# noahchalifour/rnnt-speech-recognition

Measured on AMD Instinct MI355X. Metric: rnnt_loss_grad_lattice_cells_per_sec, higher is better.
Workload: dtype f32

## Files before the change

rnnt-speech-recognition_amd/csrc/rnnt_common.h:

```cpp
#pragma once
#include <hip/hip_runtime.h>
#include <stdint.h>

#include <type_traits>

namespace rnnt {

constexpr float kNeg = -1.0e30f;
constexpr float kNegTest = -1.0e29f;
constexpr float kLog2e = 1.4426950408889634f;
constexpr float kLn2 = 0.6931471805599453f;
constexpr int kRebase = 8;

struct FastDiv {
    uint32_t d, m, s;
};
inline FastDiv make_fastdiv(uint32_t d) {
    FastDiv f;
    f.d = d;
    uint32_t s = 0;
    while ((1ull << s) < d) ++s;
    f.s = s;
    f.m = (uint32_t)((((1ull << s) - d) << 32) / d) + 1u;
    return f;
}
__device__ __forceinline__ uint32_t fdiv(uint32_t n, const FastDiv f) {
    return (__umulhi(n, f.m) + n) >> f.s;
}

struct TileGeom {
    int TT, UU, tiles_t, tiles_u, cpr;
    FastDiv div_tu, div_tt, divUU, div_cpr, divTT;
};

struct LossParams {
    const float *acts;
    float *grads;
    const int *labels;
    const int *label_lengths;
    const int *input_lengths;
    const float *cost_scale;
    float *costs;
    float *lse;
    float *W;
    float *A;
    float *Bt;
    float *offA;
    float *offB;
    double *ll;
    int *EA;
    int *EB;
    float *lik;
    int *flags;
    int NCl;
    float2 *pstat;
    int *lshift;
    int *bar;
    int nPstat;
    int pstatStride;
    int B, T, U, V, blank;
    int b0, nb;
    int visit_all;
    int precise;
    int N, Nr, Up, NC, NG;
    uint32_t cells;
    FastDiv divU, divT, divV, divOG;
    TileGeom tile;
    float fe_lambda;
};

struct WsLayout {
    size_t lse, W, A, Bt, offA, offB, ll, EA, EB, lik, flags, pstat, lshift, bar, total;
    int NCl, nPstat;
    int N, Nr, Up, NC, NG, OG;
};

inline size_t align_up(size_t x, size_t a) { return (x + a - 1) / a * a; }

constexpr int kMaxU = 8192;
inline int sweep_K(int U) {
    const int k = (U + 63) / 64;
    const int avail[] = {1, 2, 3, 4, 6, 8, 12, 16};
    for (int a : avail)
        if (k <= a) return a;
    return 0;
}
template <int K, int G>
struct SweepRing {
    static constexpr size_t kChunk = (size_t)G * 2 * 64 * K * sizeof(float);
    static constexpr int NB = (4 * kChunk + 16 <= 128 * 1024) ? 4 : 3;
    static constexpr size_t kBytes = NB * kChunk + 16;
    static_assert(kBytes <= 160 * 1024, "chunk ring exceeds the LDS");
};
template <typename F>
inline hipError_t sweep_dispatch(int U, F &&f) {
    using std::integral_constant;
    switch (sweep_K(U)) {
        case 1: return f(integral_constant<int, 1>(), integral_constant<int, 16>());
        case 2: return f(integral_constant<int, 2>(), integral_constant<int, 16>());
        case 3: return f(integral_constant<int, 3>(), integral_constant<int, 16>());
        case 4: return f(integral_constant<int, 4>(), integral_constant<int, 16>());
        case 6: return f(integral_constant<int, 6>(), integral_constant<int, 8>());
        case 8: return f(integral_constant<int, 8>(), integral_constant<int, 8>());
        case 12: return f(integral_constant<int, 12>(), integral_constant<int, 4>());
        case 16: return f(integral_constant<int, 16>(), integral_constant<int, 4>());
        default: return hipErrorInvalidValue;
    }
}
constexpr int kFillByte = 0xF1;

inline WsLayout make_layout(int T, int U, int B) {
    WsLayout w;
    w.N = T + U - 1;
    w.Nr = (int)align_up((size_t)w.N, 16);
    w.Up = sweep_K(U) ? 64 * sweep_K(U) : (int)align_up((size_t)U, 64);
    w.NC = w.Nr / kRebase + 1;
    w.OG = sweep_K(U) ? sweep_K(U) : 64;
    w.NG = w.Up / w.OG;
    size_t off = 0;
    auto take = [&](size_t bytes) {
        size_t o = off;
        off = align_up(off + bytes, 256);
        return o;
    };
    w.lse = take((size_t)B * T * U * sizeof(float));
    w.W = take((size_t)B * w.Nr * 2 * w.Up * sizeof(float));
    w.A = take((size_t)B * w.Nr * w.Up * sizeof(float));
    w.Bt = take((size_t)B * w.Nr * w.Up * sizeof(float));
    w.offA = take((size_t)B * w.NC * w.NG * sizeof(float));
    w.offB = take((size_t)B * w.NC * w.NG * sizeof(float));
    w.ll = take((size_t)B * 2 * sizeof(double));
    w.NCl = w.Nr / 4 + 1;
    w.EA = take((size_t)B * w.NCl * 64 * sizeof(int));
    w.EB = take((size_t)B * w.NCl * 64 * sizeof(int));
    w.lik = take((size_t)B * 4 * sizeof(float));
    w.flags = take((size_t)B * 4 * sizeof(int));
    {
        const int nu = (U + 31) / 32, UU = (U + nu - 1) / nu, TT = (256 / UU) > T ? T : (256 / UU);
        w.nPstat = ((T + TT - 1) / TT) * ((U + UU - 1) / UU) * 4;
    }
    w.pstat = take((size_t)B * w.nPstat * 2 * sizeof(float));
    w.lshift = take((size_t)B * sizeof(int));
    w.bar = take((size_t)B * 8 * sizeof(int));
    w.total = off;
    return w;
}

inline TileGeom make_tile(int T, int U, int V) {
    TileGeom g;
    const int nu = (U + 31) / 32;
    g.UU = (U + nu - 1) / nu;
    g.TT = 256 / g.UU;
    if (g.TT > T) g.TT = T;
    g.tiles_u = (U + g.UU - 1) / g.UU;
    g.tiles_t = (T + g.TT - 1) / g.TT;
    g.cpr = g.UU * V / 4;
    g.div_tu = make_fastdiv((uint32_t)g.tiles_u);
    g.div_tt = make_fastdiv((uint32_t)g.tiles_t);
    g.divUU = make_fastdiv((uint32_t)g.UU);
    g.divTT = make_fastdiv((uint32_t)(g.TT > 0 ? g.TT : 1));
    g.div_cpr = make_fastdiv((uint32_t)(g.cpr > 0 ? g.cpr : 1));
    return g;
}

constexpr float kExpTabLimit = 43.0f;
constexpr float kExpTab2Log2e = 2.8853900817779268f;
#ifdef __HIPCC__
__device__ __forceinline__ float exp_tab(float x) { return __builtin_amdgcn_exp2f(x * kExpTab2Log2e); }
__device__ __forceinline__ bool exp_tab_out_of_range(float x) { return !(fabsf(x) <= kExpTabLimit); }
#endif

constexpr int kHookBlocks = 1024;
struct JointHooks {
    int prep_mode;
    int prefilled;
    unsigned *dmax_enc;
    unsigned *dmax_pred;
};

#ifdef __HIPCC__
__device__ __forceinline__ void lds_dma16(const void *global, void *lds) {
    __builtin_amdgcn_global_load_lds((__attribute__((address_space(1))) const void *)global, (__attribute__((address_space(3))) void *)lds, 16, 0, 0);
}
#endif

inline int device_cu_count() {
    int dev = 0, n = 0;
    if (hipGetDevice(&dev) != hipSuccess) return 256;
    if (hipDeviceGetAttribute(&n, hipDeviceAttributeMultiprocessorCount, dev) != hipSuccess || n <= 0) return 256;
    return n;
}
template <typename Kernel>
inline hipError_t set_lds(Kernel kernel, size_t bytes) {
    if (bytes <= 64 * 1024) return hipSuccess;
    return hipFuncSetAttribute((const void *)kernel, hipFuncAttributeMaxDynamicSharedMemorySize, (int)bytes);
}

hipError_t launch_fill(void *dst, int byte, size_t bytes, hipStream_t s);
hipError_t launch_fill2(void *dst0, int byte0, size_t bytes0, void *dst1, int byte1, size_t bytes1, hipStream_t s);

bool tile_path_ok(const LossParams &p, bool grad);
hipError_t launch_lsm(const LossParams &p, hipStream_t s);
hipError_t launch_sweeps(const LossParams &p, hipStream_t s);
hipError_t launch_grad(const LossParams &p, hipStream_t s);
bool lin_path_ok(const LossParams &p);
hipError_t launch_lsm_lin(const LossParams &p, hipStream_t s);
hipError_t launch_sweeps_lin(const LossParams &p, hipStream_t s);
hipError_t launch_grad_lin(const LossParams &p, hipStream_t s);
hipError_t launch_redo_lin(const LossParams &p, bool force, hipStream_t s);

}
```

rnnt-speech-recognition_amd/csrc/rnnt_entrypoint.hip:

```cpp
#include "../../include/rnnt.h"
#include "rnnt_common.h"
#include "rnnt_lin.h"
#include "rnnt_align.h"
#include "rnnt_host.h"

using namespace rnnt;

namespace rnnt {
hipError_t joint_workspace_bytes(int T, int U, int B, int J, int V, int joint_dtype, size_t *bytes);
hipError_t joint_f16_backward_rows(void *workspace, int T, int U, int B, int J, int V, int rows[2], hipStream_t s);
hipError_t joint_backward_rows(void *workspace, int T, int U, int B, int J, int V, int rows[2], hipStream_t s);
hipError_t launch_joint_loss(const float *enc_proj, const float *pred_proj, const float *W2, const float *b2,
                             const int *labels, const int *label_lengths, const int *input_lengths,
                             const float *cost_scale, int J, int V, int B, int T, int U, int blank, float *costs,
                             float *d_enc_proj, float *d_pred_proj, float *dW2, float *db2, int joint_dtype,
                             int phases, void *workspace, hipStream_t s, const JointHooks *hooks, float fe_lambda);
hipError_t joint_aux_pointers(void *workspace, int T, int U, int B, int J, int V, float **expE, float **expP, float **tflag);
hipError_t launch_joint_prefill(void *workspace, int T, int U, int B, int J, int V, hipStream_t s);
bool joint_dtype_supported(int joint_dtype, int J, int V);
bool dense_supported(int H, int J);
hipError_t dense_workspace_bytes(int B, int T, int U, int H, int J, size_t base, size_t *bytes);
void dense_proj_pointers(void *workspace, int B, int T, int U, int H, int J, size_t base, float **enc_proj, float **pred_proj,
                         float **d_enc_proj, float **d_pred_proj);
void dense_hook_pointers(void *workspace, int B, int T, int U, int H, int J, size_t base, unsigned **dmax_enc, unsigned **dmax_pred);
// ... 27 lines not shown
                                    int Tc, int K, int N, int joint_dtype, bool timed, void *workspace, hipStream_t s);
hipError_t launch_beam_stream_feed(const float *enc, int Te, const int *chunk_frames, const int *reset, const int *final_, int H, int J,
                                   int V, int S, int Tc, int K, int N, int joint_dtype, bool timed, void *workspace, hipStream_t s);
bool prednet_layout_ok(const rnntPrednetBlock *blocks, int L, int E, int V, int Jp, int R, size_t *bytes);
hipError_t launch_prednet_begin(const float *emb, const rnntPrednetBlock *blocks, int L, int E, int V, const float *W1, int Jp, int R,
                                float *out, void *workspace, hipStream_t s);
hipError_t launch_prednet_step(const int *emitted, const int *parents, float *out, const rnntPrednetBlock *blocks, int L, int E,
                               int V, int Jp, int R, void *workspace, hipStream_t s);
bool encoder_layout_ok(const rnntPrednetBlock *blocks, int L, int F, float bn_eps, int ridx, int f, int R, int Tmax, size_t *bytes);
hipError_t launch_encoder_begin(const rnntPrednetBlock *blocks, int L, int F, const float *bn_mean, const float *bn_var,
                                const float *bn_weight, const float *bn_bias, float bn_eps, int ridx, int f, int R, int Tmax,
                                void *workspace, hipStream_t s);
hipError_t launch_encoder_run(const float *x, int T, float *out, const rnntPrednetBlock *blocks, int L, int F, float bn_eps, int ridx,
                              int f, int R, int Tmax, void *workspace, hipStream_t s);
hipError_t launch_encoder_run_rows(const float *x, int T, const int *row_frames, const int *reset, float *out,
                                   const rnntPrednetBlock *blocks, int L, int F, float bn_eps, int ridx, int f, int R, int Tmax,
                                   void *workspace, hipStream_t s);
bool lstm_train_layout_ok(int R, int T, int H, int P, bool proj, size_t *bytes);
hipError_t launch_lstm_train_fwd(float *gates, const float *W_hh, const float *W_hr, float *y, float *c, float *h, int R, int T, int H,
                                 int P, void *workspace, hipStream_t s);
hipError_t launch_lstm_train_bwd(float *gates, const float *c, const float *dy, const float *W_hh, const float *W_hr, float *dr, int R,
                                 int T, int H, int P, void *workspace, hipStream_t s);
hipError_t launch_prednet_reset(const int *reset, float *out, const rnntPrednetBlock *blocks, int L, int E, int V, int Jp, int R,
                                void *workspace, hipStream_t s);
hipError_t greedy_stream_workspace_bytes(int Tc, int S, int H, int J, int V, int joint_dtype, size_t *bytes);
hipError_t launch_greedy_stream_begin(const float *W1, const float *b1, const float *W2, const float *b2, int H, int J, int V, int S,
                                      int Tc, int joint_dtype, void *workspace, hipStream_t s);
hipError_t launch_greedy_stream_feed(const float *enc, int Te, const int *chunk_frames, const int *reset, const int *final_,
                                     const int *max_symbols, int max_per_frame, int *hyp_lengths, float *scores, int *all_done,
                                     int *frame_base, int H, int J, int V, int S, int Tc, int joint_dtype, void *workspace,
                                     hipStream_t s);
bool frontend_layout_ok(int K, int S, int L, int step, int M, int stack, int rm, size_t *bytes, int *max_rows);
hipError_t launch_frontend_begin(const float *window, const float *mel_weights, int K, int S, int L, int step, int M, int stack,
                                 int rm, void *workspace, hipStream_t s);
hipError_t launch_frontend_feed(const float *audio, int cs, const int *samples, const int *reset, const int *final_, int norm,
                                float *rows, int *counts, int K, int S, int L, int step, int M, int stack, int rm, void *workspace,
                                hipStream_t s);
}

static rnntStatus_t check_options(const rnntOptions &o) {
    if (o.loc != RNNT_GPU) return RNNT_STATUS_INVALID_VALUE;
    if (!o.batch_first) return RNNT_STATUS_INVALID_VALUE;
    if (o.maxT <= 0 || o.maxU <= 0 || o.blank_label < 0) return RNNT_STATUS_INVALID_VALUE;
    if (o.maxU > kMaxU) return RNNT_STATUS_INVALID_VALUE;
    return RNNT_STATUS_SUCCESS;
}

static bool fill_params(LossParams &p, const float *acts, float *grads, const int *labels,
                        const int *label_lengths, const int *input_lengths, const float *cost_scale, int V,
                        int B, float *costs, void *workspace, const rnntOptions &o) {
    const long long cells = (long long)B * o.maxT * o.maxU;
    if (cells <= 0 || cells >= (1ll << 31)) return false;
    if (((uintptr_t)workspace & 255) != 0) return false;
    const WsLayout w = make_layout(o.maxT, o.maxU, B);
    char *ws = (char *)workspace;
    p.acts = acts;
    p.grads = grads;
    p.labels = labels;
    p.label_lengths = label_lengths;
    p.input_lengths = input_lengths;
    p.cost_scale = cost_scale;
    p.costs = costs;
    p.lse = (float *)(ws + w.lse);
    p.W = (float *)(ws + w.W);
    p.A = (float *)(ws + w.A);
    p.Bt = (float *)(ws + w.Bt);
    p.offA = (float *)(ws + w.offA);
    p.offB = (float *)(ws + w.offB);
    p.ll = (double *)(ws + w.ll);
    p.EA = (int *)(ws + w.EA);
    p.EB = (int *)(ws + w.EB);
    p.lik = (float *)(ws + w.lik);
    p.flags = (int *)(ws + w.flags);
    p.NCl = w.NCl;
    p.pstat = (float2 *)(ws + w.pstat);
    p.lshift = (int *)(ws + w.lshift);
    p.bar = (int *)(ws + w.bar);
    p.nPstat = w.nPstat;
    p.pstatStride = 4;
    p.B = B, p.T = o.maxT, p.U = o.maxU, p.V = V, p.blank = o.blank_label;
    p.b0 = 0, p.nb = B;
    p.precise = 0;
    p.visit_all = 0;
    p.fe_lambda = 0.f;
    p.tile = make_tile(o.maxT, o.maxU, V);
    p.N = w.N, p.Nr = w.Nr, p.Up = w.Up, p.NC = w.NC, p.NG = w.NG;
    p.cells = (uint32_t)cells;
    p.divU = make_fastdiv((uint32_t)o.maxU);
    p.divT = make_fastdiv((uint32_t)o.maxT);
    p.divV = make_fastdiv((uint32_t)V);
    p.divOG = make_fastdiv((uint32_t)w.OG);
    return true;
}

namespace rnnt {
bool fill_loss_params(LossParams &p, const float *acts, float *grads, const int *labels, const int *label_lengths,
                      const int *input_lengths, const float *cost_scale, int V, int B, float *costs, void *workspace,
                      int maxT, int maxU, int blank) {
    rnntOptions o;
    o.loc = RNNT_GPU, o.stream = nullptr, o.blank_label = blank, o.maxT = maxT, o.maxU = maxU, o.batch_first = true;
    return fill_params(p, acts, grads, labels, label_lengths, input_lengths, cost_scale, V, B, costs, workspace, o);
}
}

extern "C" {

int get_warprnnt_version(void) { return 1; }

const char *rnntGetStatusString(rnntStatus_t status) {
    switch (status) {
        case RNNT_STATUS_SUCCESS: return "no error";
        case RNNT_STATUS_MEMOPS_FAILED: return "hip memcpy or memset failed";
        case RNNT_STATUS_INVALID_VALUE: return "invalid value";
        case RNNT_STATUS_EXECUTION_FAILED: return "execution failed";
        case RNNT_STATUS_UNKNOWN_ERROR:
        default: return "unknown error";
    }
}

rnntStatus_t get_workspace_size(int maxT, int maxU, int minibatch, bool gpu, size_t *size_bytes) {
    if (!size_bytes || maxT <= 0 || maxU <= 0 || minibatch <= 0 || !gpu) return RNNT_STATUS_INVALID_VALUE;
    *size_bytes = make_layout(maxT, maxU, minibatch).total;
    return RNNT_STATUS_SUCCESS;
}

static rnntStatus_t run_forward(LossParams &p, const WsLayout &w, hipStream_t s) {
    if (lin_path_ok(p)) {
        hipError_t e = launch_lsm_lin(p, s);
        if (e != hipSuccess) return from_hip(e);
        return from_hip(launch_sweeps_lin(p, s));
    }
    if (!tile_path_ok(p, false) && launch_fill(p.W, kFillByte, w.A - w.W, s) != hipSuccess) return RNNT_STATUS_MEMOPS_FAILED;
    p.precise = 1;
    hipError_t e = launch_lsm(p, s);
    if (e != hipSuccess) return from_hip(e);
    return from_hip(launch_sweeps(p, s));
}

static rnntStatus_t validate(const void *acts, const void *labels, const void *ll, const void *il, const void *ws,
                      int V, int B, const rnntOptions &o) {
    if (!acts || !labels || !ll || !il || !ws) return RNNT_STATUS_INVALID_VALUE;
    if (V <= 0 || B <= 0) return RNNT_STATUS_INVALID_VALUE;
    rnntStatus_t st = check_options(o);
    if (st != RNNT_STATUS_SUCCESS) return st;
    if (o.blank_label >= V) return RNNT_STATUS_INVALID_VALUE;
    return RNNT_STATUS_SUCCESS;
}

rnntStatus_t compute_rnnt_loss_fwd(const float *acts, const int *flat_labels, const int *label_lengths,
                                   const int *input_lengths, int alphabet_size, int minibatch, float *costs,
                                   void *workspace, rnntOptions options) {
    if (!costs) return RNNT_STATUS_INVALID_VALUE;
    rnntStatus_t st = validate(acts, flat_labels, label_lengths, input_lengths, workspace, alphabet_size, minibatch,
                               options);
    if (st != RNNT_STATUS_SUCCESS) return st;
    LossParams p;
    if (!fill_params(p, acts, nullptr, flat_labels, label_lengths, input_lengths, nullptr, alphabet_size,
                     minibatch, costs, workspace, options))
        return RNNT_STATUS_INVALID_VALUE;
    hipStream_t s = (hipStream_t)options.stream;
    const WsLayout w = make_layout(options.maxT, options.maxU, minibatch);
    st = run_forward(p, w, s);
    if (st != RNNT_STATUS_SUCCESS || !lin_path_ok(p)) return st;
    return from_hip(launch_redo_lin(p, false, s));
}

static rnntStatus_t run_backward(LossParams &p, hipStream_t s) {
    if (!lin_path_ok(p)) return from_hip(launch_grad(p, s));
    const bool patch = tile_path_ok(p, true);
    if (patch) {
        hipError_t e = launch_grad_lin(p, s);
        if (e != hipSuccess) return from_hip(e);
    }
    return from_hip(launch_redo_lin(p, !patch, s));
}

rnntStatus_t compute_rnnt_loss_bwd(const float *acts, float *grads, const int *flat_labels,
                                   const int *label_lengths, const int *input_lengths, const float *cost_scale,
                                   int alphabet_size, int minibatch, void *workspace, rnntOptions options) {
    if (!grads) return RNNT_STATUS_INVALID_VALUE;
    rnntStatus_t st = validate(acts, flat_labels, label_lengths, input_lengths, workspace, alphabet_size, minibatch,
                               options);
    if (st != RNNT_STATUS_SUCCESS) return st;
    LossParams p;
    if (!fill_params(p, acts, grads, flat_labels, label_lengths, input_lengths, cost_scale, alphabet_size,
                     minibatch, nullptr, workspace, options))
        return RNNT_STATUS_INVALID_VALUE;
    return run_backward(p, (hipStream_t)options.stream);
}

static bool fastemit_ok(float lambda) { return lambda >= 0.f && lambda <= 1.f; }

static rnntStatus_t loss_flags_call(const float *acts, float *grads, const int *flat_labels,
                                    const int *label_lengths, const int *input_lengths, const float *cost_scale,
                                    int alphabet_size, int minibatch, float *costs, void *workspace,
                                    const rnntOptions &options, unsigned int flags, float fastemit_lambda) {
    if (flags & ~(unsigned)RNNT_VISIT_ALL) return RNNT_STATUS_INVALID_VALUE;
    if (!grads)
        return compute_rnnt_loss_fwd(acts, flat_labels, label_lengths, input_lengths, alphabet_size, minibatch,
                                     costs, workspace, options);
    rnntStatus_t st = validate(acts, flat_labels, label_lengths, input_lengths, workspace, alphabet_size, minibatch,
                               options);
    if (st != RNNT_STATUS_SUCCESS) return st;
    LossParams p;
    if (!fill_params(p, acts, grads, flat_labels, label_lengths, input_lengths, cost_scale, alphabet_size,
                     minibatch, costs, workspace, options))
        return RNNT_STATUS_INVALID_VALUE;
    p.visit_all = (flags & RNNT_VISIT_ALL) ? 1 : 0;
    p.fe_lambda = fastemit_lambda;
    hipStream_t s = (hipStream_t)options.stream;
    if (costs) {
        const WsLayout w = make_layout(options.maxT, options.maxU, minibatch);
        st = run_forward(p, w, s);
        if (st != RNNT_STATUS_SUCCESS) return st;
    }
    return run_backward(p, s);
}

rnntStatus_t compute_rnnt_loss_flags(const float *acts, float *grads, const int *flat_labels,
                                     const int *label_lengths, const int *input_lengths, const float *cost_scale,
                                     int alphabet_size, int minibatch, float *costs, void *workspace,
                                     rnntOptions options, unsigned int flags) {
    return loss_flags_call(acts, grads, flat_labels, label_lengths, input_lengths, cost_scale, alphabet_size, minibatch, costs,
                           workspace, options, flags, 0.f);
}

rnntStatus_t compute_rnnt_loss_fastemit(const float *acts, float *grads, const int *flat_labels,
                                        const int *label_lengths, const int *input_lengths, const float *cost_scale,
                                        int alphabet_size, int minibatch, float *costs, void *workspace,
                                        rnntOptions options, unsigned int flags, float fastemit_lambda) {
    if (!fastemit_ok(fastemit_lambda)) return RNNT_STATUS_INVALID_VALUE;
    return loss_flags_call(acts, grads, flat_labels, label_lengths, input_lengths, cost_scale, alphabet_size, minibatch, costs,
                           workspace, options, flags, fastemit_lambda);
}

rnntStatus_t compute_rnnt_loss_ex(const float *acts, float *grads, const int *flat_labels,
                                  const int *label_lengths, const int *input_lengths, const float *cost_scale,
                                  int alphabet_size, int minibatch, float *costs, void *workspace,
                                  rnntOptions options) {
    if (grads && !costs) return RNNT_STATUS_INVALID_VALUE;
    return compute_rnnt_loss_flags(acts, grads, flat_labels, label_lengths, input_lengths, cost_scale, alphabet_size, minibatch,
                                   costs, workspace, options, 0u);
}

rnntStatus_t compute_rnnt_loss(const float *acts, float *grads, const int *flat_labels,
                               const int *label_lengths, const int *input_lengths, int alphabet_size,
                               int minibatch, float *costs, void *workspace, rnntOptions options) {
    return compute_rnnt_loss_ex(acts, grads, flat_labels, label_lengths, input_lengths, nullptr, alphabet_size,
                                minibatch, costs, workspace, options);
}

rnntStatus_t get_joint_workspace_size(int maxT, int maxU, int minibatch, int joint_size, int alphabet_size,
                                      size_t *size_bytes) {
    if (!size_bytes || maxT <= 0 || maxU <= 0 || minibatch <= 0 || joint_size <= 0 || alphabet_size <= 0)
        return RNNT_STATUS_INVALID_VALUE;
    return from_hip(joint_workspace_bytes(maxT, maxU, minibatch, joint_size, alphabet_size, -1, size_bytes));
}

static rnntStatus_t joint_call(const float *enc_proj, const float *pred_proj, const float *W2, const float *b2,
                               const int *flat_labels, const int *label_lengths, const int *input_lengths,
                               const float *cost_scale, int joint_size, int alphabet_size, int minibatch, float *costs,
                               float *d_enc_proj, float *d_pred_proj, float *dW2, float *db2, int joint_dtype,
                               int phases, void *workspace, const rnntOptions &options, float fastemit_lambda = 0.f) {
    if (!enc_proj || !pred_proj || !W2 || !b2 || !flat_labels || !label_lengths || !input_lengths || !workspace)
        return RNNT_STATUS_INVALID_VALUE;
    if ((phases & 1) && !costs) return RNNT_STATUS_INVALID_VALUE;
    if (joint_size <= 0 || alphabet_size <= 0 || minibatch <= 0) return RNNT_STATUS_INVALID_VALUE;
    rnntStatus_t st = check_options(options);
    if (st != RNNT_STATUS_SUCCESS) return st;
    if (options.blank_label >= alphabet_size) return RNNT_STATUS_INVALID_VALUE;
    if (options.maxU > 1024) return RNNT_STATUS_INVALID_VALUE;
    if (joint_dtype & ~(0xff | RNNT_VISIT_ALL)) return RNNT_STATUS_INVALID_VALUE;
    if (joint_dtype & RNNT_VISIT_ALL) phases |= 8;
    joint_dtype &= 0xff;
    if (!joint_dtype_supported(joint_dtype, joint_size, alphabet_size)) return RNNT_STATUS_INVALID_VALUE;
    const bool any_grad = d_enc_proj || d_pred_proj || dW2 || db2;
    if (any_grad && !(d_enc_proj && d_pred_proj && dW2 && db2)) return RNNT_STATUS_INVALID_VALUE;
    if ((phases & 2) && !(phases & 1) && !any_grad) return RNNT_STATUS_INVALID_VALUE;
    return from_hip(launch_joint_loss(enc_proj, pred_proj, W2, b2, flat_labels, label_lengths, input_lengths,
                                      cost_scale, joint_size, alphabet_size, minibatch, options.maxT, options.maxU,
                                      options.blank_label, costs, d_enc_proj, d_pred_proj, dW2, db2, joint_dtype,
                                      phases, workspace, (hipStream_t)options.stream, nullptr, fastemit_lambda));
}

rnntStatus_t compute_rnnt_joint_loss(const float *enc_proj, const float *pred_proj, const float *W2,
                                     const float *b2, const int *flat_labels, const int *label_lengths,
                                     const int *input_lengths, const float *cost_scale, int joint_size,
                                     int alphabet_size, int minibatch, float *costs, float *d_enc_proj,
                                     float *d_pred_proj, float *dW2, float *db2, int joint_dtype, void *workspace,
                                     rnntOptions options) {
    return joint_call(enc_proj, pred_proj, W2, b2, flat_labels, label_lengths, input_lengths, cost_scale, joint_size,
                      alphabet_size, minibatch, costs, d_enc_proj, d_pred_proj, dW2, db2, joint_dtype, 3, workspace,
                      options);
// ... 855 lines not shown
```

rnnt-speech-recognition_amd/csrc/rnnt_kernels.hip:

```cpp
#include "rnnt_common.h"
#include "rnnt_cell.h"
#include "rnnt_sweep.h"
#include "rnnt_cellwave.h"
#include "rnnt_lin.h"
#include "rnnt_cellbody.h"

#include <float.h>
#include <math.h>
#include <stdlib.h>

namespace rnnt {


typedef float gs_v4f __attribute__((ext_vector_type(4)));
__device__ __forceinline__ void grad_store16(gs_v4f *dst, const gs_v4f v) { __builtin_nontemporal_store(v, dst); }

constexpr int kFillRows = 16;

template <int VP, bool GRAD, bool AL = true, bool LIN = false, bool FE = false>
__global__ __launch_bounds__(256) void cell_tile_kernel(const LossParams p) {
    extern __shared__ __attribute__((aligned(16))) float lds[];
    const int tid = threadIdx.x;
    const int lane = tid & 63;
    const int wave = __builtin_amdgcn_readfirstlane(tid >> 6);
    const int V = p.V;
    const TileGeom &tg = p.tile;
    const uint32_t n_patch_wg = (uint32_t)p.nb * (uint32_t)tg.tiles_t * (uint32_t)tg.tiles_u;
    uint32_t vblock = blockIdx.x;
    if (!GRAD) {
        const uint32_t per = (uint32_t)p.Nr / kFillRows, n_fill = (uint32_t)p.nb * per;
        const uint32_t pgs = (n_patch_wg + 7u) >> 3, fgs = (n_fill + 7u) >> 3, P = (pgs + fgs) / fgs;
        const uint32_t g = blockIdx.x >> 3, l8 = blockIdx.x & 7u;
        const uint32_t k = g / P;
        const bool is_fill = g - k * P == P - 1u && k < fgs;
        if (is_fill) {
            const uint32_t f = k * 8u + l8;
            if (f >= n_fill) return;
            const int fb = p.b0 + (int)(f / per), chunk = (int)(f % per);
            const int Tf = length_T(p, fb), Uf = length_U(p, fb);
            const int Nf = Tf + Uf - 1;
            float2 *Wb = (float2 *)p.W + (size_t)fb * p.Nr * p.Up;
            const float2 z = LIN ? make_float2(0.f, 0.f) : make_float2(kNeg, kNeg);
            for (int idx = tid; idx < kFillRows * p.Up; idx += 256) {
                const int rr = idx / p.Up, u = idx - rr * p.Up;
                const int n = chunk * kFillRows + rr;
                if (n < Nf && (u < max(0, n - Tf + 1) || u > min(n, Uf - 1))) Wb[(size_t)n * p.Up + u] = z;
            }
            return;
        }
        vblock = (g - min(k, fgs)) * 8u + l8;
        if (vblock >= n_patch_wg) return;
    }
    uint32_t bid;
    {
        const uint32_t nwg = n_patch_wg, xcd = vblock & 7u, idx = vblock >> 3;
        const uint32_t q = nwg >> 3, r = nwg & 7u;
        bid = (xcd < r ? xcd * (q + 1u) : r * (q + 1u) + (xcd - r) * q) + idx;
        if (GRAD) bid = (xcd < r ? xcd * (q + 1u) : r * (q + 1u) + (xcd - r) * q) + ((xcd < r ? q + 1u : q) - 1u - idx);
    }
    const uint32_t q1 = fdiv(bid, tg.div_tu);
    const uint32_t tu = bid - q1 * (uint32_t)tg.tiles_u;
    const uint32_t bb = fdiv(q1, tg.div_tt);
    const uint32_t tt = q1 - bb * (uint32_t)tg.tiles_t;
    const int b = p.b0 + (int)bb;
    const int t0 = (int)tt * tg.TT, u0 = (int)tu * tg.UU;
    const int Tb = length_T(p, b), Ub = length_U(p, b);
    if (GRAD && LIN && lin_skip(p, b)) return;

    const int rows_valid = max(0, min(tg.TT, Tb - t0));
    const int cols_valid = max(0, min(tg.UU, Ub - u0));
    const int rows_in = max(0, min(tg.TT, p.T - t0));
    const int cols_in = max(0, min(tg.UU, p.U - u0));
    const int q_valid = cols_valid * V / 4;
    const int q_in = cols_in * V / 4;
    const int row_lds = AL ? tg.UU * V : ((tg.UU * V + 3 + 3) & ~3);
    const size_t row_f = (size_t)p.U * V;
    const size_t patch0 = ((size_t)(b * p.T + t0) * p.U + u0) * V;

    auto store_row = [&](const int r, const float *src) {
        const size_t s0 = patch0 + r * row_f;
        if (AL) {
            for (int q = lane; q < q_in; q += 64) {
                typedef float v4f __attribute__((ext_vector_type(4)));
                const v4f v = src ? ((const v4f *)src)[q] : (v4f){0.f, 0.f, 0.f, 0.f};
                grad_store16((v4f *)(p.grads + s0 + q * 4), v);
            }
        } else {
            const int a = (int)(s0 & 3), len = cols_in * V;
            float *base = p.grads + (s0 - a);
            for (int q = lane; q * 4 < a + len; q += 64) {
                const int e0 = q * 4 - a;
                typedef float v4f __attribute__((ext_vector_type(4)));
                const v4f vv = src ? ((const v4f *)src)[q] : (v4f){0.f, 0.f, 0.f, 0.f};
                const float v[4] = {vv[0], vv[1], vv[2], vv[3]};
                if (e0 >= 0 && e0 + 3 < len) {
                    grad_store16((v4f *)(base + q * 4), vv);
                } else {
#pragma unroll
                    for (int k = 0; k < 4; ++k)
                        if (e0 + k >= 0 && e0 + k < len) base[q * 4 + k] = v[k];
                }
            }
        }
    };

    float2 *const pslot = p.pstat + (size_t)b * p.nPstat + ((size_t)tt * tg.tiles_u + tu) * 4 + wave;
    if (rows_valid == 0 || cols_valid == 0) {
        if (GRAD) {
            for (int r = wave; r < rows_in; r += 4) store_row(r, nullptr);
        }
        if (!GRAD && LIN && lane == 0) *pslot = make_float2(0.f, 0.f);
        return;
    }

    const uint32_t r = fdiv((uint32_t)tid, tg.divUU);
    const int cu = tid - (int)r * tg.UU;
    Cell cl;
    cl.b = b, cl.t = t0 + (int)r, cl.u = u0 + cu, cl.Tb = Tb, cl.Ub = Ub;
    cl.valid = ((int)r < rows_valid) && (cu < cols_valid);
    const uint32_t c = ((uint32_t)(b * p.T + cl.t)) * (uint32_t)p.U + (uint32_t)cl.u;

    LinGrad lg = {};
    uint32_t lword = ~0u;
    if (GRAD && LIN) {
        bool live = false;
        if (cl.valid) {
            lg = lin_grad_setup(p, cl);
            if (lg.bad) atomicOr(p.flags + 4 * cl.b + kFlagG, 1);
            live = p.visit_all || !(lg.l2occ <= (float)-kOccFloorWave);
            cl.valid = live;
        }
        const uint64_t m = __ballot(live);
        const int ncell = tg.TT * tg.UU, nw = (ncell + 31) >> 5;
        uint32_t *const lw = (uint32_t *)lds;
        if (lane == 0 && wave * 64 < ncell) lw[2 * wave] = (uint32_t)m;
        if (lane == 0 && wave * 64 + 32 < ncell) lw[2 * wave + 1] = (uint32_t)(m >> 32);
        __syncthreads();
        lword = lane < nw ? lw[lane] : 0u;
        __syncthreads();
        if (__ballot(lword != 0u) == 0) {
            for (int rr = wave; rr < rows_in; rr += 4) store_row(rr, nullptr);
            return;
        }
    }
    auto cells_live = [&](const int klo, const int khi) -> bool {
        const uint32_t wlo = (uint32_t)__shfl((int)lword, klo >> 5), whi = (uint32_t)__shfl((int)lword, khi >> 5);
        const uint64_t bits = ((uint64_t)whi << 32 | wlo) >> (klo & 31);
        return (bits & ((2ull << (khi - klo)) - 1ull)) != 0;
    };

    for (int r = wave; r < rows_valid; r += 4) {
        const size_t s0 = patch0 + r * row_f;
        const int a = AL ? 0 : (int)(s0 & 3);
        const float *src = p.acts + (s0 - a);
        float *dst = lds + r * row_lds;
        const int nq = AL ? q_valid : (a + cols_valid * V + 3) / 4;
        for (int q0 = 0; q0 < nq; q0 += 64) {
            const int q = q0 + lane;
            bool need = q < nq;
            if (GRAD && LIN) {
                const int e = min(q, nq - 1) * 4 - a;
                const int lo = (int)fdiv((uint32_t)max(0, e), p.divV), hi = AL ? lo : (int)fdiv((uint32_t)min(e + 3, cols_valid * V - 1), p.divV);
                need = cells_live(r * tg.UU + lo, r * tg.UU + hi) && need;
            }
            if (need) {
                __builtin_amdgcn_global_load_lds((glb_void *)(src + q * 4), (lds_void *)(dst + q0 * 4), 16, 0, 0);
            }
        }
    }
    wait_vm0();
    __syncthreads();

    float stat = 0.f;
    if (AL) {
        if ((GRAD && tid < tg.TT * tg.UU) || cl.valid) stat = cell_body<VP, true, GRAD, LIN, false, FE>(p, cl, c, lds + tid * V, lds + tid * V, &lg);
    } else if ((int)r < tg.TT) {
        const int a = (int)((patch0 + r * row_f) & 3);
        if (GRAD || cl.valid) stat = cell_body<VP, false, GRAD, LIN, false, FE>(p, cl, c, lds + r * row_lds + a + cu * V, lds + r * row_lds + a + cu * V, &lg);
    }
    if (!GRAD && LIN) {
        float cnt = cl.valid ? 1.f : 0.f;
        stat = cl.valid ? stat : 0.f;
#pragma unroll
        for (int off = 32; off > 0; off >>= 1) stat += __shfl_xor(stat, off), cnt += __shfl_xor(cnt, off);
        if (lane == 0) *pslot = make_float2(stat, cnt);
        __syncthreads();
        float2 *const Wp = (float2 *)p.W + ((size_t)b * p.Nr + t0 + u0) * p.Up + u0;
        const uint32_t total = (uint32_t)(tg.TT + tg.UU - 1) * (uint32_t)tg.TT;
        for (uint32_t j = tid; j < total; j += 256) {
            const uint32_t d = fdiv(j, tg.divTT);
            const int rr = (int)(j - d * (uint32_t)tg.TT), cc = (int)d - rr;
// ... 290 lines not shown
```

rnnt-speech-recognition_amd/csrc/rnnt_lin.h:

```cpp
#pragma once
#include "rnnt_sweep.h"

namespace rnnt {

__host__ __device__ constexpr int lin_shift_max(int K) { return (K == 1 || K >= 12) ? 2 : 3; }
constexpr float kLinDecayBits = 6.2f;
constexpr int kLinDrag = 118;
constexpr int kFrameNone = -(1 << 28);
constexpr int kCertBits = -40;
constexpr float kTinyEdge = 7.8886091e-31f;

enum { kFlagA = 0, kFlagB = 1, kFlagG = 2, kFlagState = 3 };

__device__ __forceinline__ void st_i32_wt(int *q, int v) { __hip_atomic_store(q, v, __ATOMIC_RELAXED, __HIP_MEMORY_SCOPE_AGENT); }
__device__ __forceinline__ float frexp_m(float x) { return __builtin_amdgcn_frexp_mantf(x); }
__device__ __forceinline__ int frexp_e(float x) { return __builtin_amdgcn_frexp_expf(x); }
__device__ __forceinline__ float ldexp_f(float x, int e) { return __builtin_ldexpf(x, e); }

__device__ __forceinline__ bool lin_skip(const LossParams &p, const int b) {
    const int *fl = p.flags + 4 * b;
    return (fl[kFlagA] | fl[kFlagB]) != 0 || fl[kFlagState] == 2;
}

template <int VP>
__device__ __forceinline__ float lin_cell_lsm(const LossParams &p, const Cell &cl, const float (&x)[VP], const float *xs) {
    float m = x[0];
#pragma unroll
    for (int i = 1; i < VP; ++i) m = fmaxf(m, x[i]);
    float s = 0.f;
    const float nml = -m * kLog2e;
#pragma unroll
    for (int i = 0; i < VP; ++i) s += ex2(fmaf(x[i], kLog2e, nml));
    const float inv = __builtin_amdgcn_rcpf(s);
    const bool blank_stays = (cl.t < cl.Tb - 1) || (cl.u == cl.Ub - 1);
    float pb = 0.f, pl = 0.f;
    if (blank_stays) {
        pb = ex2(fmaf(xs[p.blank], kLog2e, nml)) * inv;
        if (!(pb >= kTinyEdge)) pb = NAN;
    }
    if (cl.u < cl.Ub - 1) {
        const int lab = clamp_label(p.labels[(size_t)cl.b * (p.U - 1) + cl.u], p.V);
        pl = ex2(fmaf(xs[lab], kLog2e, nml)) * inv;
        if (!(pl >= kTinyEdge)) pl = NAN;
    }
    float *const xo = const_cast<float *>(xs);
    xo[0] = pb, xo[1] = pl;
    const float best = fmaxf(pb, pl);
    return (pb != pb || pl != pl) ? 200.f : -lg2(fmaxf(best, 1.0e-37f));
}

struct LinGrad {
    float h0;
    float hb;
    float hl;
    float l2occ;
    bool has_blank_corr, has_label, bad;
    int lab;
};

__device__ __forceinline__ LinGrad lin_grad_setup(const LossParams &p, const Cell &cl) {
    LinGrad g;
    const int n = cl.t + cl.u;
    const size_t sk = ((size_t)cl.b * p.Nr + n) * p.Up + cl.u;
    const float ma = p.A[sk], mb = p.Bt[sk];
    const int sh = p.lshift[cl.b];
    const int kc = n >> sh, kc1 = (n + 1) >> sh;
    const int l0 = (int)fdiv((uint32_t)cl.u, p.divOG), l1 = (int)fdiv((uint32_t)cl.u + 1u, p.divOG);
    const size_t tb = (size_t)cl.b * p.NCl * 64;
    const int ea = p.EA[tb + (size_t)kc * 64 + l0], eb = p.EB[tb + (size_t)kc * 64 + l0];
    const float mL = p.lik[4 * cl.b];
    const int EL = ((const int *)p.lik)[4 * cl.b + 1];
    const float scale = p.cost_scale ? p.cost_scale[cl.b] : 1.0f;
    const int xa = frexp_e(ma), xb = frexp_e(mb);
    const float qa = scale * frexp_m(ma) * __builtin_amdgcn_rcpf(mL);
    const int base = ea + xa - EL;
    g.h0 = ldexp_f(qa * frexp_m(mb), base + eb + xb);
    g.l2occ = lg2(frexp_m(ma) * frexp_m(mb) * __builtin_amdgcn_rcpf(mL)) + (float)(ea + xa + eb + xb - EL);
    g.has_blank_corr = true;
    g.hb = 0.f;
    if (cl.t < cl.Tb - 1) {
        const float m1 = p.Bt[sk + p.Up];
        g.hb = ldexp_f(qa * frexp_m(m1), base + p.EB[tb + (size_t)kc1 * 64 + l0] + frexp_e(m1));
    } else if (cl.u == cl.Ub - 1) {
        g.hb = ldexp_f(qa, base);
    } else {
        g.has_blank_corr = false;
    }
    g.has_label = cl.u < cl.Ub - 1;
    g.lab = 0;
    g.hl = 0.f;
    if (g.has_label) {
        g.lab = clamp_label(p.labels[(size_t)cl.b * (p.U - 1) + cl.u], p.V);
        const float m1 = p.Bt[sk + p.Up + 1];
        g.hl = ldexp_f(qa * frexp_m(m1), base + p.EB[tb + (size_t)kc1 * 64 + l1] + frexp_e(m1));
    }
    int worst = ea + eb - 252 - EL;
    if (mb != 0.f) worst = max(worst, ea - 126 + eb + xb - EL);
    if (ma != 0.f) worst = max(worst, eb - 126 + ea + xa - EL);
    g.bad = worst > kCertBits || !(ma <= FLT_MAX) || !(mb <= FLT_MAX) || !(ma >= 0.f) || !(mb >= 0.f);
    return g;
}

}
```

rnnt-speech-recognition_amd/csrc/rnnt_lin_kernels.hip:

```cpp
#include "rnnt_common.h"
#include "rnnt_cell.h"
#include "rnnt_sweep.h"
#include "rnnt_cellwave.h"
#include "rnnt_lin.h"
#include "rnnt_cellbody.h"
#include "rnnt_redo.h"

namespace rnnt {

__device__ __forceinline__ float dpp_lower_zero(float x) {
    return __int_as_float(__builtin_amdgcn_update_dpp(0, __float_as_int(x), 0x138 , 0xf, 0xf, true));
}
__device__ __forceinline__ float dpp_upper_zero(float x) {
    return __int_as_float(__builtin_amdgcn_update_dpp(0, __float_as_int(x), 0x130 , 0xf, 0xf, true));
}
__device__ __forceinline__ int dpp_lower_i(int x, int fill) {
    return __builtin_amdgcn_update_dpp(fill, x, 0x138, 0xf, 0xf, false);
}
__device__ __forceinline__ int dpp_upper_i(int x, int fill) {
    return __builtin_amdgcn_update_dpp(fill, x, 0x130, 0xf, 0xf, false);
}

struct LinState {
    int E;
// ... 238 lines not shown
            lin_issue_row<K, 1>(wq[1], abase);
            lin_alpha_fast_steps<K, G, SH, 0>(a, wq, abase, st, voff, lane, r0);
        } else {
            for (int i = 0; i < G; ++i) {
                const int n = r0 + i + 1;
                if (n > last_row) break;
                LinRow<K> wc;
                lin_load_row<K>(wc, cur + i * 2 * Up);
                lin_alpha_step<K>(a, wc, st.d);
                if ((n & ((1 << SH) - 1)) == 0) lin_renorm<K, false, SH>(a, st, n >> SH);
                store_diag<K, false>(st.row, voff, lane, a);
                st.row += Up;
            }
        }
        if (ck + 1 < nchunks) {
            asm volatile("s_waitcnt lgkmcnt(0)" ::: "memory");
            if (lane == 0) lds_post(lk.consumed, ck + 1);
        }
    }
    {
        const float *wrow = bufs + ((nchunks - 1) % NB) * chunkf + (last_row % G) * 2 * Up + 2 * u0;
#pragma unroll
        for (int j = 0; j < K; ++j)
            if (u0 + j == Ub - 1) lin_record(p, b, 0, a[j] * wrow[2 * j], st.E, timed_out);
    }
}

template <int K, int G, int NB, int SH>
__device__ void lin_beta_sweep(const LossParams &p, float *bufs, const LdLink lk, const int b, const int lane) {
    constexpr int Up = 64 * K, chunkf = G * 2 * Up;
    const int Tb = length_T(p, b), Ub = length_U(p, b);
    const int Nb = Tb + Ub - 1;
    float *out = p.Bt + (size_t)b * p.Nr * Up;
    const int voff = lane * K * 4;
    const int u0 = lane * K;

    float bv[K];
#pragma unroll
    for (int j = 0; j < K; ++j) bv[j] = (u0 + j == Ub - 1) ? 1.f : 0.f;
    const int last = Nb - 1;
    const int ckl = last / G;
    LinState st;
    st.E = 0, st.d = 0;
    st.tab = p.EB + (size_t)b * p.NCl * 64 + lane;
    st.row = out + (size_t)last * Up;

    LandedView lv;
    lv.addr0 = lk.landed;
#pragma unroll
    for (int w = 0; w < kLinLoaders; ++w) lv.have[w] = 0;
    bool timed_out = lengths_invalid(p, b);
    for (int ck = ckl; ck >= 0; --ck) {
        const int i_ring = ckl - ck;
        timed_out |= !lv.wait(i_ring);
        const float *cur = bufs + (i_ring % NB) * chunkf + 2 * u0;
        const int r0 = ck * G;
        if (r0 + G - 1 < last) {
            const uint32_t abase = (uint32_t)(uintptr_t)((lds_void *)cur);
            LinRow<K> wq[3];
            lin_issue_row<K, G - 1>(wq[0], abase);
            lin_issue_row<K, G - 2>(wq[1], abase);
            lin_beta_fast_steps<K, G, SH, 0>(bv, wq, abase, st, voff, lane, r0);
        } else {
            for (int ii = 0; ii < G; ++ii) {
                const int i = G - 1 - ii;
                const int n = r0 + i;
                if (n > last) continue;
                LinRow<K> wc;
                lin_load_row<K>(wc, cur + i * 2 * Up);
                lin_beta_step<K>(bv, wc, st.d);
                if ((n & ((1 << SH) - 1)) == (1 << SH) - 1 || n == last) lin_renorm<K, true, SH>(bv, st, n >> SH);
                store_diag<K, false>(st.row, voff, lane, bv);
                st.row -= Up;
            }
        }
        if (ck > 0) {
            asm volatile("s_waitcnt lgkmcnt(0)" ::: "memory");
            if (lane == 0) lds_post(lk.consumed, i_ring + 1);
        }
    }
    if (lane == 0) lin_record(p, b, 1, bv[0], st.E, timed_out);
}

template <int K, int G, int NB>
__global__ __launch_bounds__(64 * (1 + kLinLoaders)) void lin_sweep_kernel(const LossParams p) {
    extern __shared__ __attribute__((aligned(16))) float lds[];
    constexpr int chunkf = G * 2 * 64 * K;
    const int tid = threadIdx.x, lane = tid & 63;
    const int wave = __builtin_amdgcn_readfirstlane(tid >> 6);
    const int b = p.b0 + (int)(blockIdx.x >> 1);
    const bool beta = (blockIdx.x & 1) != 0;
    int *ctr = (int *)(lds + NB * chunkf);
    if (tid < 2 * kLinLoaders) ctr[tid] = 0;
    __syncthreads();
    LdLink lk;
    lk.landed = (uint32_t)(uintptr_t)((lds_void *)ctr);
    lk.consumed = lk.landed + 4u;
    if (wave >= 1) {
        LdLink mine = lk;
        mine.landed = lk.landed + 8u * (uint32_t)(wave - 1);
        if (beta)
            sweep_loader<K, G, NB, true, kLinLoaders>(p, lds, mine, b, lane, wave - 1);
        else
            sweep_loader<K, G, NB, false, kLinLoaders>(p, lds, mine, b, lane, wave - 1);
    } else {
        constexpr int SHmax = lin_shift_max(K);
        int sh = SHmax;
        if constexpr (SHmax > 2) {
            float sum = 0.f, cnt = 0.f;
            const float2 *ps = p.pstat + (size_t)b * p.nPstat;
            const int stride = p.pstatStride, npatch = p.nPstat / stride;
            for (int i0 = 0; i0 < npatch; i0 += 512) {
                float2 q[8];
#pragma unroll
                for (int k = 0; k < 8; ++k) {
                    const int i = i0 + 64 * k + lane;
                    q[k] = (i < npatch) ? ps[(size_t)stride * i] : make_float2(0.f, 0.f);
                }
#pragma unroll
                for (int k = 0; k < 8; ++k) sum += q[k].x, cnt += q[k].y;
            }
#pragma unroll
            for (int off = 32; off > 0; off >>= 1) sum += __shfl_xor(sum, off), cnt += __shfl_xor(cnt, off);
            sh = (sum > kLinDecayBits * cnt) ? 2 : SHmax;
            sh = __builtin_amdgcn_readfirstlane(sh);
        }
        if constexpr (SHmax > 2) {
            if (sh == 2) {
                if (beta)
                    lin_beta_sweep<K, G, NB, 2>(p, lds, lk, b, lane);
                else
                    lin_alpha_sweep<K, G, NB, 2>(p, lds, lk, b, lane);
                return;
            }
        }
        if (beta)
            lin_beta_sweep<K, G, NB, SHmax>(p, lds, lk, b, lane);
        else
            lin_alpha_sweep<K, G, NB, SHmax>(p, lds, lk, b, lane);
    }
}

template <int K, int G, int NB, bool FE = false>
__global__ __launch_bounds__(kRedoThreads) void lin_redo_kernel(const LossParams p, const int force, const int team) {
    extern __shared__ __attribute__((aligned(16))) float lds[];
    constexpr int chunkf = G * 2 * 64 * K;
    const int tid = threadIdx.x;
    const int ub = (int)blockIdx.x / team;
    const int b = p.b0 + ub;
    RedoTeam tm;
    tm.k = (int)blockIdx.x - ub * team, tm.n = team, tm.bar = p.bar + kRedoCtr * b, tm.ok = true;
    int *fl = p.flags + 4 * b;
    typedef int i32x4 __attribute__((ext_vector_type(4)));
    typedef double f64x2 __attribute__((ext_vector_type(2)));
    const i32x4 fw = __builtin_nontemporal_load((const i32x4 *)fl);
    const f64x2 lw = __builtin_nontemporal_load((const f64x2 *)(p.ll + 2 * b));
    const int state = fw[kFlagState];
    bool redo = false;
    if (state != 2) {
        const bool agree = fabs(lw[0] - lw[1]) * 0.6931471805599453 <= 2e-5 + 1e-8 * fabs(lw[0]);
        redo = force || (fw[kFlagA] | fw[kFlagB] | fw[kFlagG]) != 0 || !agree;
        if (!redo) return;
    } else if (!p.grads) {
        return;
    }
    if (redo) redo_lattice<K, G, NB>(p, b, tm, lds, tid);
    uint32_t lo, hi;
    redo_cell_range(p, b, tm, lo, hi);
    if (p.grads) redo_cells<true, FE>(p, lo, hi, tid, lds, NB * chunkf);
    if (!tm.ok) {
        if (p.costs && tm.k == 0 && tid == 0) st_f32_wt(p.costs + b, NAN);
        if (p.grads)
            for (size_t i = (size_t)lo * p.V + tid; i < (size_t)hi * p.V; i += kRedoThreads) p.grads[i] = NAN;
    }
}

bool lin_path_ok(const LossParams &p) { return p.V >= 2 && sweep_K(p.U) >= 1 && tile_path_ok(p, false); }

template <int K, int G>
static hipError_t launch_lin_sweep(const LossParams &p, hipStream_t s) {
    using R = SweepRing<K, G>;
    static_assert(2 * kLinLoaders * sizeof(int) <= 16, "the loaders' flag words exceed the ring's 16 bytes");
    hipError_t e = set_lds(lin_sweep_kernel<K, G, R::NB>, R::kBytes);
    if (e != hipSuccess) return e;
    hipLaunchKernelGGL((lin_sweep_kernel<K, G, R::NB>), dim3(2 * p.nb), dim3(64 * (1 + kLinLoaders)), R::kBytes, s, p);
    return hipGetLastError();
}
template <int K, int G, bool FE = false>
static hipError_t launch_lin_redo(const LossParams &p, const bool force, hipStream_t s) {
    using R = SweepRing<K, G>;
    hipError_t e = set_lds(lin_redo_kernel<K, G, R::NB, FE>, R::kBytes);
    if (e != hipSuccess) return e;
    const int team = redo_team_size(p.nb, p.T, p.U, device_cu_count());
    hipLaunchKernelGGL((lin_redo_kernel<K, G, R::NB, FE>), dim3(p.nb * team), dim3(kRedoThreads), R::kBytes, s, p, force ? 1 : 0, team);
    return hipGetLastError();
}

hipError_t launch_sweeps_lin(const LossParams &p, hipStream_t s) {
    return sweep_dispatch(p.U, [&](auto K, auto G) { return launch_lin_sweep<K, G>(p, s); });
}
hipError_t launch_redo_lin(const LossParams &p, const bool force, hipStream_t s) {
    if (p.grads && p.fe_lambda != 0.f)
        return sweep_dispatch(p.U, [&](auto K, auto G) { return launch_lin_redo<K, G, true>(p, force, s); });
    return sweep_dispatch(p.U, [&](auto K, auto G) { return launch_lin_redo<K, G>(p, force, s); });
}

}
```

Before: 14.11 billion.

## Zero padded gradient patches in idle blocks during the linear sweep

Adds extra blocks to the lin sweep launch, one per CU left free beyond the 2*nb sweep blocks. These blocks write zeros to gradient tiles that lie entirely outside each sequence's valid T/U extent, and the later grad kernel skips storing those tiles. The intent is to overlap this padding-fill store traffic with the latency-bound alpha/beta sweeps on otherwise idle CUs. The cost is a more complex launch, a new prezero flag, and duplicated validity logic that must agree between the two kernels.

```diff
diff --git a/rnnt-speech-recognition_amd/csrc/rnnt_common.h b/rnnt-speech-recognition_amd/csrc/rnnt_common.h
--- a/rnnt-speech-recognition_amd/csrc/rnnt_common.h
+++ b/rnnt-speech-recognition_amd/csrc/rnnt_common.h
@@ -61,6 +61,7 @@
     int B, T, U, V, blank;
     int b0, nb;
     int visit_all;
+    int prezero;
     int precise;
     int N, Nr, Up, NC, NG;
     uint32_t cells;
@@ -204,6 +205,7 @@
 hipError_t launch_sweeps(const LossParams &p, hipStream_t s);
 hipError_t launch_grad(const LossParams &p, hipStream_t s);
 bool lin_path_ok(const LossParams &p);
+int lin_fill_groups(int nb);
 hipError_t launch_lsm_lin(const LossParams &p, hipStream_t s);
 hipError_t launch_sweeps_lin(const LossParams &p, hipStream_t s);
 hipError_t launch_grad_lin(const LossParams &p, hipStream_t s);
diff --git a/rnnt-speech-recognition_amd/csrc/rnnt_entrypoint.hip b/rnnt-speech-recognition_amd/csrc/rnnt_entrypoint.hip
--- a/rnnt-speech-recognition_amd/csrc/rnnt_entrypoint.hip
+++ b/rnnt-speech-recognition_amd/csrc/rnnt_entrypoint.hip
@@ -133,6 +133,7 @@
     p.b0 = 0, p.nb = B;
     p.precise = 0;
     p.visit_all = 0;
+    p.prezero = 0;
     p.fe_lambda = 0.f;
     p.tile = make_tile(o.maxT, o.maxU, V);
     p.N = w.N, p.Nr = w.Nr, p.Up = w.Up, p.NC = w.NC, p.NG = w.NG;
@@ -260,6 +261,7 @@
     p.visit_all = (flags & RNNT_VISIT_ALL) ? 1 : 0;
     p.fe_lambda = fastemit_lambda;
     hipStream_t s = (hipStream_t)options.stream;
+    p.prezero = (costs && !p.visit_all && lin_path_ok(p) && tile_path_ok(p, true) && lin_fill_groups(p.nb) > 0) ? 1 : 0;
     if (costs) {
         const WsLayout w = make_layout(options.maxT, options.maxU, minibatch);
         st = run_forward(p, w, s);
diff --git a/rnnt-speech-recognition_amd/csrc/rnnt_kernels.hip b/rnnt-speech-recognition_amd/csrc/rnnt_kernels.hip
--- a/rnnt-speech-recognition_amd/csrc/rnnt_kernels.hip
+++ b/rnnt-speech-recognition_amd/csrc/rnnt_kernels.hip
@@ -11,9 +11,6 @@
 
 namespace rnnt {
 
-
-typedef float gs_v4f __attribute__((ext_vector_type(4)));
-__device__ __forceinline__ void grad_store16(gs_v4f *dst, const gs_v4f v) { __builtin_nontemporal_store(v, dst); }
 
 constexpr int kFillRows = 16;
 
@@ -106,7 +103,7 @@
 
     float2 *const pslot = p.pstat + (size_t)b * p.nPstat + ((size_t)tt * tg.tiles_u + tu) * 4 + wave;
     if (rows_valid == 0 || cols_valid == 0) {
-        if (GRAD) {
+        if (GRAD && !(LIN && lin_prezero(p, (int)tt, (int)tu, p.input_lengths[b], p.label_lengths[b]))) {
             for (int r = wave; r < rows_in; r += 4) store_row(r, nullptr);
         }
         if (!GRAD && LIN && lane == 0) *pslot = make_float2(0.f, 0.f);
diff --git a/rnnt-speech-recognition_amd/csrc/rnnt_lin.h b/rnnt-speech-recognition_amd/csrc/rnnt_lin.h
--- a/rnnt-speech-recognition_amd/csrc/rnnt_lin.h
+++ b/rnnt-speech-recognition_amd/csrc/rnnt_lin.h
@@ -21,6 +21,17 @@
     const int *fl = p.flags + 4 * b;
     return (fl[kFlagA] | fl[kFlagB]) != 0 || fl[kFlagState] == 2;
 }
+
+__host__ __device__ inline bool lin_prezero_patch(const int tt, const int tu, const TileGeom &tg, const int Tb, const int Ub) {
+    return tt * tg.TT >= Tb || tu * tg.UU >= Ub;
+}
+__device__ __forceinline__ bool lin_prezero(const LossParams &p, const int tt, const int tu, const int il, const int ll) {
+    if (p.prezero == 0 || il < 1 || il > p.T || ll < 0 || ll > p.U - 1) return false;
+    return lin_prezero_patch(tt, tu, p.tile, il, ll + 1);
+}
+
+typedef float gs_v4f __attribute__((ext_vector_type(4)));
+__device__ __forceinline__ void grad_store16(gs_v4f *dst, const gs_v4f v) { __builtin_nontemporal_store(v, dst); }
 
 template <int VP>
 __device__ __forceinline__ float lin_cell_lsm(const LossParams &p, const Cell &cl, const float (&x)[VP], const float *xs) {
diff --git a/rnnt-speech-recognition_amd/csrc/rnnt_lin_kernels.hip b/rnnt-speech-recognition_amd/csrc/rnnt_lin_kernels.hip
--- a/rnnt-speech-recognition_amd/csrc/rnnt_lin_kernels.hip
+++ b/rnnt-speech-recognition_amd/csrc/rnnt_lin_kernels.hip
@@ -344,11 +344,63 @@
     if (lane == 0) lin_record(p, b, 1, bv[0], st.E, timed_out);
 }
 
+__device__ __forceinline__ void lin_prezero_fill(const LossParams &p, const uint32_t k, const uint32_t n, const int tid) {
+    const TileGeom &tg = p.tile;
+    const int V = p.V;
+    const uint32_t total = (uint32_t)p.nb * (uint32_t)tg.tiles_t * (uint32_t)tg.tiles_u;
+    const size_t row_f = (size_t)p.U * V;
+    const bool al = (V & 3) == 0;
+    const gs_v4f z = {0.f, 0.f, 0.f, 0.f};
+    int blk = -1, v_il = 0, v_ll = 0;
+    for (uint32_t pi = k; pi < total; pi += n) {
+        const uint32_t q1 = fdiv(pi, tg.div_tu);
+        const uint32_t tu = pi - q1 * (uint32_t)tg.tiles_u;
+        const uint32_t bb = fdiv(q1, tg.div_tt);
+        const uint32_t tt = q1 - bb * (uint32_t)tg.tiles_t;
+        const int b = p.b0 + (int)bb;
+        if ((int)(bb >> 6) != blk) {
+            blk = (int)(bb >> 6);
+            const int i = p.b0 + min(64 * blk + (tid & 63), p.nb - 1);
+            v_il = p.input_lengths[i], v_ll = p.label_lengths[i];
+            asm volatile("" : "+v"(v_il), "+v"(v_ll));
+        }
+        if (!lin_prezero(p, (int)tt, (int)tu, __builtin_amdgcn_readlane(v_il, (int)(bb & 63u)), __builtin_amdgcn_readlane(v_ll, (int)(bb & 63u)))) continue;
+        const int t0 = (int)tt * tg.TT, u0 = (int)tu * tg.UU;
+        const int rows_in = max(0, min(tg.TT, p.T - t0));
+        const int cols_in = max(0, min(tg.UU, p.U - u0));
+        const size_t patch0 = ((size_t)(b * p.T + t0) * p.U + u0) * V;
+        for (int r = 0; r < rows_in; ++r) {
+            const size_t s0 = patch0 + r * row_f;
+            if (al) {
+                const int q_in = cols_in * V / 4;
+                for (int q = tid; q < q_in; q += 64 * (1 + kLinLoaders)) grad_store16((gs_v4f *)(p.grads + s0 + q * 4), z);
+            } else {
+                const int a = (int)(s0 & 3), len = cols_in * V;
+                float *base = p.grads + (s0 - a);
+                for (int q = tid; q * 4 < a + len; q += 64 * (1 + kLinLoaders)) {
+                    const int e0 = q * 4 - a;
+                    if (e0 >= 0 && e0 + 3 < len) {
+                        grad_store16((gs_v4f *)(base + q * 4), z);
+                    } else {
+#pragma unroll
+                        for (int i = 0; i < 4; ++i)
+                            if (e0 + i >= 0 && e0 + i < len) base[q * 4 + i] = 0.f;
+                    }
+                }
+            }
+        }
+    }
+}
+
 template <int K, int G, int NB>
 __global__ __launch_bounds__(64 * (1 + kLinLoaders)) void lin_sweep_kernel(const LossParams p) {
     extern __shared__ __attribute__((aligned(16))) float lds[];
     constexpr int chunkf = G * 2 * 64 * K;
     const int tid = threadIdx.x, lane = tid & 63;
+    if (blockIdx.x >= 2u * (uint32_t)p.nb) {
+        lin_prezero_fill(p, blockIdx.x - 2u * (uint32_t)p.nb, gridDim.x - 2u * (uint32_t)p.nb, tid);
+        return;
+    }
     const int wave = __builtin_amdgcn_readfirstlane(tid >> 6);
     const int b = p.b0 + (int)(blockIdx.x >> 1);
     const bool beta = (blockIdx.x & 1) != 0;
@@ -439,13 +491,16 @@
 
 bool lin_path_ok(const LossParams &p) { return p.V >= 2 && sweep_K(p.U) >= 1 && tile_path_ok(p, false); }
 
+int lin_fill_groups(const int nb) { return max(0, device_cu_count() - 2 * nb); }
+
 template <int K, int G>
 static hipError_t launch_lin_sweep(const LossParams &p, hipStream_t s) {
     using R = SweepRing<K, G>;
     static_assert(2 * kLinLoaders * sizeof(int) <= 16, "the loaders' flag words exceed the ring's 16 bytes");
     hipError_t e = set_lds(lin_sweep_kernel<K, G, R::NB>, R::kBytes);
     if (e != hipSuccess) return e;
-    hipLaunchKernelGGL((lin_sweep_kernel<K, G, R::NB>), dim3(2 * p.nb), dim3(64 * (1 + kLinLoaders)), R::kBytes, s, p);
+    const int n_fill = p.prezero ? lin_fill_groups(p.nb) : 0;
+    hipLaunchKernelGGL((lin_sweep_kernel<K, G, R::NB>), dim3(2 * p.nb + n_fill), dim3(64 * (1 + kLinLoaders)), R::kBytes, s, p);
     return hipGetLastError();
 }
 template <int K, int G, bool FE = false>
```

After: 14.17 billion, median of 6. Within noise of the previous version (+0.4%).
